# Hypersonic-cpu/DSP-AudioRecLabs

Hardware: AMD Instinct MI355X
Metric: frames/sec (framing+window+E/M/ZCR) on 1 s 44.1 kHz clips; 1/2/4/8 GPU (higher is better)
Workload: dtype fp32

## Files before the change

dsp-audioreclabs_amd/csrc/extract.hip:

```cpp
#include <hip/hip_runtime.h>
#include <stdint.h>

#include <algorithm>

#include "dsp_audiorec.h"
#include "extract_layout.h"
#include "dsp_device.h"

#ifndef DSP_ABL
#define DSP_ABL 0
#endif

namespace dsp {

static constexpr int NT = EXTRACT_THREADS;
static constexpr int NWAVE = NT / 64;
static constexpr int RREG = EXTRACT_RREG;
static constexpr int NRV = 4 * RREG;

#ifdef DSP_STAMPS
#define STAMP(clip, k)                                                                           \
    do {                                                                                         \
        if (threadIdx.x == 0 && p.stamps) p.stamps[(size_t)(clip) * 32 + (k)] = __builtin_amdgcn_s_memtime(); \
    } while (0)
// ... 26 lines not shown
#define MARK(name) \
    do {           \
    } while (0)
#endif

struct ExtractParams {
    const int16_t *pcm;
    const int64_t *offsets;
    int B, ncap, L, S;
    const double *window;
    int do_vad;
    double hi, lo, zr;
    float *feat;
    int32_t *start_end, *n_frames, *status;
    int ostride;
    double *vad_energy;
    int32_t *vad_zcr;
    int ld_vad;
    float *seq;
    int ld_seq;
    unsigned long long *stamps;
    unsigned *queue;
    int qchunk;
    ExtractCarve cv;
};

static_assert(__is_standard_layout(ExtractParams) && __is_trivially_copyable(ExtractParams),
              "ExtractParams is a plain kernel argument block");
static_assert(sizeof(ExtractParams) <= 1024, "kernel argument block");

struct ClipStatsRaw {
    double mq, Mp, invM2;
    float invMf;
    int tpos, t0, nv, kneg;
};
struct Shared {
    long long red_k[NWAVE];
    int red_a[NWAVE], red_b[NWAVE];
    double pa, pb;
    ClipStatsRaw cs;
    double noise_e, noise_z;
    double oslo[3], oshi[3];
    int n3, n1, n6, exact, j0, j1, next;
    int qnext, qend, qcursor, qrange;
    int cdir, cy;
    unsigned smask;
    int schunk;
    int sclear;
    long long noff[2];
    int noff_for;
};
static_assert(sizeof(Shared) <= EXTRACT_SHARED_BYTES, "grow EXTRACT_SHARED_BYTES");
static_assert((EXTRACT_OSTAGE & (EXTRACT_OSTAGE - 1)) == 0 && EXTRACT_OSTAGE <= 32, "chunk of 2^k <= 32 clips");

struct ClipRef {
    int64_t base;
    int lead, n, nvec, nword;
    bool ok;
};

__device__ __forceinline__ ClipRef clip_ref_at(const ExtractParams &p, int64_t o0, int64_t o1)
{
    ClipRef c;
    const int64_t nn = o1 - o0;
    c.ok = nn > 0 && nn <= p.ncap;
    c.n = c.ok ? (int)nn : 0;
    c.base = o0 & ~(int64_t)7;
    c.lead = (int)(o0 - c.base);
    c.nvec = c.ok ? (c.lead + c.n + 7) >> 3 : 0;
    c.nword = (c.lead + c.n + 31) >> 5;
    return c;
}
__device__ __forceinline__ ClipRef clip_ref(const ExtractParams &p, int i)
{
    return clip_ref_at(p, p.offsets[i], p.offsets[i + 1]);
}
__device__ __forceinline__ ClipRef clip_none()
{
    ClipRef c;
    c.base = 0;
    c.lead = c.n = c.nvec = c.nword = 0;
    c.ok = false;
    return c;
}

struct Ctx {
    Shared *sh;
    const float *wtab;
    uint32_t *posw;
    unsigned long long *wS2;
    int *wS1;
    double *vE;
    int32_t *vZ;
    float *fE, *fM;
    int32_t *fZ;
    uint16_t *zw;
    int *ztot;
    int *rank;
    int *pS1;
    unsigned long long *pS2;
    int32_t *orow;
    int64_t total;
    int stamp_clip;
};

__device__ __forceinline__ __amdgpu_buffer_rsrc_t clip_rsrc(const ExtractParams &p, const ClipRef &c)
{
    return __builtin_amdgcn_make_buffer_rsrc(const_cast<int16_t *>(p.pcm + c.base), 0, c.nvec * 16, 0x00020000);
}
__device__ __forceinline__ short8 load_vec(const ExtractParams &p, const ClipRef &c, int v)
{
    return __builtin_bit_cast(short8, __builtin_amdgcn_raw_buffer_load_b128(clip_rsrc(p, c), 16 * v, 0, 0));
}
__device__ __forceinline__ short8 load_cvec(const ExtractParams &p, const ClipRef &c, int v)
{
    return __builtin_bit_cast(short8, __builtin_amdgcn_raw_buffer_load_b128(clip_rsrc(p, c), 2 * c.lead + 16 * v, 0, 0));
}
__device__ __forceinline__ void issue_clip(short8 (&regs)[NRV], const ExtractParams &p, const ClipRef &c,
                                           int tid = (int)threadIdx.x, int r0 = 0, int r1 = RREG)
{
    const __amdgpu_buffer_rsrc_t rs = clip_rsrc(p, c);
    const int voff = 64 * tid;
#pragma unroll
    for (int r = r0; r < r1; r++)
#pragma unroll
        for (int k = 0; k < 4; k++)
            regs[4 * r + k] = __builtin_bit_cast(
                short8, __builtin_amdgcn_raw_buffer_load_b128(rs, voff + 16 * k, 64 * NT * r, 0));
}
__device__ __forceinline__ int opaque_tid()
{
    int t = (int)threadIdx.x;
    asm volatile("" : "+v"(t));
    return t;
}

__device__ __forceinline__ void vad_noise(const Ctx &c, int nv, int lane)
{
    const double *vE = c.vE;
    const int32_t *vZ = c.vZ;
    const int nfr = min(5, nv / 10);
    double noise_e, noise_z;
    if (nfr > 0) {
        long long zs = 0;
        for (int q = 0; q < nfr; q++) zs += vZ[q] + vZ[nv - nfr + q];
        auto cat = [&](int q) { return q < nfr ? vE[q] : vE[nv - 2 * nfr + q]; };
        noise_e = np_small_sum(cat, 2 * nfr) / (double)(2 * nfr);
        noise_z = (double)zs / (double)(2 * nfr);
    } else {
        double me = INFINITY;
        int mz = 0x7fffffff;
        for (int q = lane; q < nv; q += 64) {
            me = fmin(me, vE[q]);
            mz = min(mz, vZ[q]);
        }
        noise_e = wave_mind(me);
        noise_z = (double)wave_min(mz);
    }
    if (lane == 0) {
        c.sh->noise_e = noise_e;
        c.sh->noise_z = noise_z;
    }
}

template <bool CERTIFY, bool FAST>
__device__ __forceinline__ int vad_scan(const ExtractParams &p, const Ctx &c, int nv, int lane)
{
    const double *vE = c.vE;
    const int32_t *vZ = c.vZ;
    Shared *sh = c.sh;
    const double noise_e = sh->noise_e, noise_z = sh->noise_z;
    const double g = p90_weight(nv);
    const double p90 = np_lerp(sh->pa, sh->pb, g);
    const ExtractParams &q = p;
    const VadThresholds th = vad_thresholds(p90, noise_e, noise_z, q);
    const double t1 = th.t1, t2 = th.t2, tz = th.tz;
    STAMP(c.stamp_clip, 10);
    int flag = 0, n3 = -1, n1 = 0, n6 = nv - 1;
    auto short_scan = [&](auto kc_t) {
        constexpr int KC = decltype(kc_t)::value;
        BitsK<KC> hiE, loE, loZ, nr1, nr2;
#pragma unroll
        for (int k = 0; k < KC; k++) {
            const int q = 64 * k + lane;
            const bool in = q < nv;
            const double e = in ? vE[q] : 0.0;
            const int z = in ? vZ[q] : 0;
            hiE.w[k] = __ballot(in && e > t1);
            loE.w[k] = __ballot(in && e <= t2);
            loZ.w[k] = __ballot(in && (double)z <= tz);
            nr1.w[k] = CERTIFY ? __ballot(in && near_tie(e, t1)) : 0ull;
            nr2.w[k] = CERTIFY ? __ballot(in && near_tie(e, t2)) : 0ull;
        }
        n3 = bits_first_ge(hiE, 0);
        const int n4 = bits_last_lt(hiE, nv);
        if (CERTIFY) {
            if (n3 < 0) flag |= bits_any_in(nr1, 0, nv);
            else flag |= bits_any_in(nr1, 0, n3 + 1) || bits_any_in(nr1, n4, nv);
        }
        if (n3 >= 0) {
            const int b2 = bits_last_lt(loE, n3);
            const int n2 = b2 >= 0 ? b2 + 1 : 0;
            const int b5 = bits_first_ge(loE, n4 + 1);
            const int n5 = b5 >= 0 ? b5 - 1 : nv - 1;
            if (CERTIFY)
                flag |= bits_any_in(nr2, max(n2 - 1, 0), n3) || bits_any_in(nr2, n4 + 1, min(n5 + 2, nv));
            const int b1 = bits_last_lt(loZ, n2);
            n1 = b1 >= 0 ? b1 + 1 : 0;
            const int b6 = bits_first_ge(loZ, n5 + 1);
            n6 = b6 >= 0 ? b6 - 1 : nv - 1;
        }
    };
    if (FAST || nv <= 128) {
        short_scan(IntT<2>());
    } else if (nv <= 256) {
        short_scan(IntT<4>());
    } else {
        int n4 = -1;
        for (int q0 = 0; q0 < nv; q0 += 64) {
            const int f = q0 + lane;
            const unsigned long long m = __ballot(f < nv && vE[f] > t1);
            if (m) {
                if (n3 < 0) n3 = q0 + __ffsll((long long)m) - 1;
                n4 = q0 + 63 - __clzll((long long)m);
            }
        }
        if (CERTIFY)
            for (int q0 = 0; q0 < nv; q0 += 64) {
                const int f = q0 + lane;
                const bool chk = f < nv && (n3 < 0 || f <= n3 || f >= n4);
                if (__ballot(chk && near_tie(vE[f], t1))) flag = 1;
            }
        if (n3 >= 0) {
            int n2 = 0, n5 = nv - 1;
            for (int q0 = ((n3 - 1) >> 6) << 6; q0 >= 0 && n3 > 0; q0 -= 64) {
                const int q = q0 + lane;
                const unsigned long long m = __ballot(q < n3 && vE[q] <= t2);
                if (m) {
                    n2 = q0 + 63 - __clzll((long long)m) + 1;
                    break;
                }
            }
            for (int q0 = ((n4 + 1) >> 6) << 6; q0 < nv; q0 += 64) {
                const int q = q0 + lane;
                const unsigned long long m = __ballot(q > n4 && q < nv && vE[q] <= t2);
                if (m) {
                    n5 = q0 + __ffsll((long long)m) - 2;
                    break;
                }
            }
            if (CERTIFY)
                for (int q0 = 0; q0 < nv; q0 += 64) {
                    const int q = q0 + lane;
                    const bool chk = q < nv && ((q >= n2 - 1 && q < n3) || (q > n4 && q <= n5 + 1));
                    if (__ballot(chk && near_tie(vE[q], t2))) flag = 1;
                }
            for (int q0 = ((n2 - 1) >> 6) << 6; q0 >= 0 && n2 > 0; q0 -= 64) {
                const int q = q0 + lane;
                const unsigned long long m = __ballot(q < n2 && (double)vZ[q] <= tz);
                if (m) {
                    n1 = q0 + 63 - __clzll((long long)m) + 1;
                    break;
                }
            }
            for (int q0 = ((n5 + 1) >> 6) << 6; q0 < nv; q0 += 64) {
                const int q = q0 + lane;
                const unsigned long long m = __ballot(q > n5 && q < nv && (double)vZ[q] <= tz);
                if (m) {
                    n6 = q0 + __ffsll((long long)m) - 2;
                    break;
                }
            }
        }
    }
    if (lane == 0) {
        sh->n3 = n3;
        sh->n1 = n1;
        sh->n6 = n6;
    }
    STAMP(c.stamp_clip, 11);
    return flag;
}

__device__ __forceinline__ int vad_partial_word(const ClipRef &cur, int L, int S, int nv, int t, int &e0, int &e1)
{
    e0 = e1 = 0;
    if (t >= 2 * nv) return -1;
    const int f = t >> 1;
    const bool end = t & 1;
    const int u0 = cur.lead + f * S, u1 = u0 + L;
    const int wa = u0 >> 5, wb = (u1 - 1) >> 5;
    if (!end && (u0 & 31)) {
        e0 = u0 & 31;
        e1 = min(32, u1 - 32 * wa);
        return wa;
    }
    if (end && (u1 & 31) && (wb != wa || !(u0 & 31))) {
        e0 = max(0, u0 - 32 * wb);
        e1 = u1 & 31;
        return wb;
    }
    return -1;
}
__device__ __forceinline__ void partial_moments_fast(const short8 (&q)[4], int e0, int e1, bool kneg, int &t1,
                                                     unsigned long long &t2)
{
    const uint32_t hi = e1 >= 32 ? ~0u : (1u << e1) - 1u;
    const uint32_t M = hi & ~((1u << e0) - 1u);
    const short2v ones = {1, 1};
    int s1 = 0;
    unsigned long long s2 = 0;
#pragma unroll
    for (int k = 0; k < 4; k++) {
        const uint32_t Mk = M >> (8 * k);
        short2v dm[4];
#pragma unroll
        for (int h = 0; h < 4; h++) {
            const uint32_t b0 = (uint32_t)__builtin_amdgcn_sbfe((int)Mk, 2 * h, 1);
            const uint32_t b1 = (uint32_t)__builtin_amdgcn_sbfe((int)Mk, 2 * h + 1, 1);
            const uint32_t m = (b0 & 0x0000FFFFu) | (b1 & 0xFFFF0000u);
            dm[h] = __builtin_bit_cast(short2v, __builtin_bit_cast(uint32_t, half_pair(q[k], h)) & m);
            s1 = __builtin_amdgcn_sdot2(dm[h], ones, s1, false);
        }
        if (kneg) {
#pragma unroll
            for (int h = 0; h < 4; h++) s2 += (unsigned)sq2(dm[h]);
        } else {
            s2 += (unsigned)sq2acc(dm[1], sq2(dm[0]));
            s2 += (unsigned)sq2acc(dm[3], sq2(dm[2]));
        }
    }
    t1 += s1;
    t2 += s2;
}

__device__ __forceinline__ int uni(int v) { return __builtin_amdgcn_readfirstlane(v); }
__device__ __forceinline__ float uni(float v)
{
    return __builtin_bit_cast(float, __builtin_amdgcn_readfirstlane(__builtin_bit_cast(int, v)));
}
__device__ __forceinline__ double uni(double v)
{
    const long long b = __builtin_bit_cast(long long, v);
    const unsigned lo = __builtin_amdgcn_readfirstlane((int)b), hi = __builtin_amdgcn_readfirstlane((int)(b >> 32));
    return __builtin_bit_cast(double, (long long)(((unsigned long long)hi << 32) | lo));
}

__device__ __forceinline__ uint64_t uni_u64(uint64_t v)
{
    const unsigned lo = __builtin_amdgcn_readfirstlane((int)v), hi = __builtin_amdgcn_readfirstlane((int)(v >> 32));
    return ((uint64_t)hi << 32) | lo;
}

struct R1Acc {
    int K, kmin, kmax;
    short2v pmin, pmax;
};
__device__ __forceinline__ R1Acc r1_acc_init()
{
    R1Acc a;
    a.K = 0;
    a.kmin = 0x7fffffff;
    a.kmax = -0x7fffffff - 1;
    a.pmin = (short2v){32767, 32767};
    a.pmax = (short2v){-32768, -32768};
    return a;
}
__device__ __forceinline__ void r1_interior(const short8 *q, int w, R1Acc &a, int *wS1, unsigned long long *wS2)
{
    int s1 = 0;
    unsigned long long s2 = 0;
    const short2v ones = {1, 1};
#pragma unroll
    for (int k = 0; k < 4; k++)
#pragma unroll
        for (int h = 0; h < 4; h += 2) {
            const short2v d0 = half_pair(q[k], h), d1 = half_pair(q[k], h + 1);
            a.pmin = __builtin_elementwise_min(a.pmin, d0);
            a.pmax = __builtin_elementwise_max(a.pmax, d0);
            a.pmin = __builtin_elementwise_min(a.pmin, d1);
            a.pmax = __builtin_elementwise_max(a.pmax, d1);
            s1 = __builtin_amdgcn_sdot2(d0, ones, s1, false);
            s1 = __builtin_amdgcn_sdot2(d1, ones, s1, false);
            s2 += (unsigned)sq2acc(d1, sq2(d0));
        }
    wS1[w] = s1;
    wS2[w] = s2;
    a.K += s1;
}
__device__ __forceinline__ void r1_redo_s2(const short8 *q, int w, unsigned long long *wS2)
{
    unsigned long long s2 = 0;
#pragma unroll
    for (int k = 0; k < 4; k++)
#pragma unroll
        for (int h = 0; h < 4; h++) s2 += (unsigned)sq2(half_pair(q[k], h));
    wS2[w] = s2;
}
__device__ __forceinline__ int r1_edge_issue(const ExtractParams &p, const ClipRef &cur, int lane)
{
    const int w = lane < 32 ? 0 : cur.nword - 1, u = 32 * w + (lane & 31);
    const bool valid = (lane < 32 || cur.nword > 1) && u >= cur.lead && u < cur.lead + cur.n;
    const int x = (short)__builtin_amdgcn_raw_buffer_load_b16(clip_rsrc(p, cur), valid ? 2 * u : 0x40000000, 0, 0);
    return valid ? x : 0x7fffffff;
}
__device__ __forceinline__ void r1_edges(int xv, int nword, int lane, R1Acc &a, int *wS1, unsigned long long *wS2)
{
    const bool valid = xv != 0x7fffffff;
    const int x = valid ? xv : 0;
    if (valid) {
        a.kmin = min(a.kmin, x);
        a.kmax = max(a.kmax, x);
    }
    a.K += x;
    const int w = lane < 32 ? 0 : nword - 1;
    if ((lane & 31) == 0 && (lane == 0 || nword > 1)) {
        int z1 = 0;
        unsigned long long z2 = 0;
        asm volatile("" : "+v"(z1), "+v"(z2));
        wS1[w] = z1;
        wS2[w] = z2;
    }
    if (valid) {
        __hip_atomic_fetch_add(wS1 + w, x, __ATOMIC_RELAXED, __HIP_MEMORY_SCOPE_WORKGROUP);
        __hip_atomic_fetch_add(wS2 + w, (unsigned long long)(unsigned)(x * x), __ATOMIC_RELAXED,
                               __HIP_MEMORY_SCOPE_WORKGROUP);
    }
}
__device__ __forceinline__ void r1_reduce_rows(const R1Acc &a, const Ctx &c, int wid, int lane)
{
    const int kmn = min(a.kmin, min((int)a.pmin.x, (int)a.pmin.y));
    const int kmx = max(a.kmax, max((int)a.pmax.x, (int)a.pmax.y));
    const int ks = dpp_row_reduce(a.K, OpAdd()), rmn = dpp_row_reduce(kmn, OpMin()), rmx = dpp_row_reduce(kmx, OpMax());
    if ((lane & 15) == 0) {
        int *rk = reinterpret_cast<int *>(c.vE);
        const int slot = 4 * wid + (lane >> 4);
        rk[slot] = ks;
        rk[32 + slot] = rmn;
        rk[64 + slot] = rmx;
    }
}
__device__ __forceinline__ uint32_t neg_byte255(const short8 &val, short2v tt, uint32_t acc)
{
    unsigned a[4];
#pragma unroll
    for (int h = 0; h < 4; h++) a[h] = __builtin_bit_cast(unsigned, __builtin_elementwise_sub_sat(half_pair(val, h), tt));
    const unsigned s03 = __builtin_amdgcn_perm(a[1], a[0], 0x0B0A0908u);
    const unsigned s47 = __builtin_amdgcn_perm(a[3], a[2], 0x0B0A0908u);
    return __builtin_amdgcn_udot4(s47, 0x80402010u, __builtin_amdgcn_udot4(s03, 0x08040201u, acc, false), false);
}
__device__ __forceinline__ uint32_t pos_word(const short8 *q, int w, int nword, int lead, int n, int tpos)
{
    const bool tbig = tpos > 32767;
    const short2v tt = {(short)(tbig ? 32767 : tpos), (short)(tbig ? 32767 : tpos)};
    const uint32_t x0 = neg_byte255(q[0], tt, 255u), x1 = neg_byte255(q[1], tt, 0u), x2 = neg_byte255(q[2], tt, 0u),
                   x3 = neg_byte255(q[3], tt, 0u);
    uint32_t P = tbig ? 0u : ((((x3 << 8) + x2) << 8) + x1 << 8) + x0;
    P = tbig ? 0u : P * 0x01010101u;
    if (w == 0 || w == nword - 1) {
        const int lo_ = min(max(lead - 32 * w, 0), 32), hi_ = min(max(lead + n - 32 * w, 0), 32);
        const uint32_t mhi = hi_ >= 32 ? ~0u : ((1u << hi_) - 1u);
        const uint32_t mlo = lo_ >= 32 ? 0u : ~((1u << lo_) - 1u);
        P &= mhi & mlo;
    }
    return P;
}

__device__ __forceinline__ int wave_incl_scan(int v)
{
    v += __builtin_amdgcn_update_dpp(0, v, 0x111, 0xF, 0xF, true);
    v += __builtin_amdgcn_update_dpp(0, v, 0x112, 0xF, 0xF, true);
    v += __builtin_amdgcn_update_dpp(0, v, 0x114, 0xF, 0xF, true);
    v += __builtin_amdgcn_update_dpp(0, v, 0x118, 0xF, 0xF, true);
    v += __builtin_amdgcn_update_dpp(0, v, 0x142, 0xA, 0xF, false);
    v += __builtin_amdgcn_update_dpp(0, v, 0x143, 0xC, 0xF, false);
    return v;
}
__device__ __forceinline__ void zseg_word(const uint16_t *zw_, const int *zt_, uint32_t P, int w, int lane, int seg)
{
    uint16_t *zw = const_cast<uint16_t *>(zw_);
    int *ztot = const_cast<int *>(zt_);
    const uint32_t nb = (uint32_t)__builtin_amdgcn_update_dpp(0, (int)P, 0x130, 0xF, 0xF, true);
    uint32_t ch = P ^ ((P >> 1) | (nb << 31));
    if (lane == 63) ch &= 0x7fffffffu;
    const int cz = __popc(ch), inc = wave_incl_scan(cz);
    zw[w] = (uint16_t)(inc - cz);
    if (lane == 63) ztot[seg] = inc;
}
__device__ __forceinline__ int zseg_count(const uint32_t *posw, const uint16_t *zw, const int *ztot, int x0, int x1)
{
    if (x1 <= x0) return 0;
    const int w0 = x0 >> 5, w1 = x1 >> 5, s0 = w0 >> 6;
    int cnt = (int)zw[w1] - (int)zw[w0] - __popc(chg_word(posw, w0) & ((1u << (x0 & 31)) - 1u));
    if (x1 & 31) cnt += __popc(chg_word(posw, w1) & ((1u << (x1 & 31)) - 1u));
    if ((w1 >> 6) != s0) cnt += ztot[s0] + (int)(chg_word(posw, 64 * s0 + 63) >> 31);
    return cnt;
}

struct ClipStats {
    double mq, Mp, invM2;
    float invMf;
    int tpos, t0, nv;
    int kneg;
};
__device__ __forceinline__ ClipStats clip_stats_rows(const Ctx &c, int lane, int n, int L, int S, int do_vad)
{
    const int *rk = reinterpret_cast<const int *>(c.vE);
    const int K = wave_sum(lane < 32 ? rk[lane] : 0);
    const int kmin = wave_min(lane < 32 ? rk[32 + lane] : 0x7fffffff);
    const int kmax = wave_max(lane < 32 ? rk[64 + lane] : -0x7fffffff - 1);
    ClipStats s;
    s.mq = uni((double)K / (double)n);
    s.Mp = uni(fmax((double)kmax - s.mq, s.mq - (double)kmin));
    s.tpos = uni((int)floor(s.mq) + 1);
    s.t0 = uni((int)floor(s.mq + 0.5));
    s.invMf = uni(s.Mp > 0.0 ? (float)(1.0 / s.Mp) : 0.0f);
    s.invM2 = uni(s.Mp > 0.0 ? 1.0 / (s.Mp * s.Mp) : 0.0);
    s.nv = (do_vad && n >= L) ? (n - L) / S + 1 : 0;
    s.kneg = kmin == -32768;
    return s;
}

__device__ __forceinline__ void p90_select_wave(const Ctx &c, int nv, int lane)
{
    const P90Rank<int> pr = p90_rank(nv);
    const int r0 = pr.r0, r1 = pr.r1;
    const bool in0 = lane < nv, in1 = lane + 64 < nv;
    const unsigned long long f0 = in0 ? dkey(c.vE[lane]) : 0ull;
    const unsigned long long f1 = in1 ? dkey(c.vE[lane + 64]) : 0ull;
    const unsigned o0 = (unsigned)(f0 >> 32), o1 = (unsigned)(f1 >> 32);
    const int d1 = nv - 1 - r1, d0 = nv - 1 - r0;
    unsigned h0 = o0, h1 = o1, ka = 0, kb = 0;
    for (int t = 0;; t++) {
        const unsigned m = wave_reduce(h0 > h1 ? h0 : h1, OpMax());
        if (t == d1) kb = m;
        if (t == d0) {
            ka = m;
            break;
        }
        const unsigned long long b0 = __ballot(h0 == m);
        if (b0) {
            if (lane == __ffsll((long long)b0) - 1) h0 = 0u;
        } else {
            if (lane == __ffsll((long long)__ballot(h1 == m)) - 1) h1 = 0u;
        }
    }
    auto full_at = [&](int r) -> double {
        const unsigned kh = r == r0 ? ka : kb;
        const unsigned long long c0 = __ballot(in0 && o0 == kh), c1 = __ballot(in1 && o1 == kh);
        if (__popcll(c0) + __popcll(c1) == 1)
            return dkey_value(c0 ? lane_read(f0, __ffsll((long long)c0) - 1)
                                 : lane_read(f1, __ffsll((long long)c1) - 1));
        const int rr = r - (__popcll(__ballot(in0 && o0 < kh)) + __popcll(__ballot(in1 && o1 < kh)));
        unsigned long long res = 0;
        for (int hh = 0; hh < 2; hh++) {
            unsigned long long cm = hh ? c1 : c0;
            while (cm) {
                const int l = __ffsll((long long)cm) - 1;
                cm &= cm - 1;
                const unsigned long long e = lane_read(hh ? f1 : f0, l);
                const int lt = __popcll(__ballot(in0 && o0 == kh && f0 < e)) + __popcll(__ballot(in1 && o1 == kh && f1 < e));
                const int eq = __popcll(__ballot(in0 && f0 == e)) + __popcll(__ballot(in1 && f1 == e));
                if (rr >= lt && rr < lt + eq) res = e;
            }
        }
        return dkey_value(res);
    };
    const double pa = full_at(r0), pb = full_at(r1);
    if (lane == 0) {
        c.sh->pa = pa;
        c.sh->pb = pb;
    }
}

__device__ __forceinline__ int vad_partial_issue(const ExtractParams &p, const ClipRef &cur, int L, int S, int nv,
                                                 int t, short8 (&qa)[4], int &e0, int &e1)
{
    const int pw = vad_partial_word(cur, L, S, nv, t, e0, e1);
    const __amdgpu_buffer_rsrc_t rs = clip_rsrc(p, cur);
    const int off = pw >= 0 ? 64 * pw : 0x40000000;
#pragma unroll
    for (int k = 0; k < 4; k++)
        qa[k] = __builtin_bit_cast(short8, __builtin_amdgcn_raw_buffer_load_b128(rs, off + 16 * k, 0, 0));
    return pw;
}

__device__ __forceinline__ void vad_frames_fast(const Ctx &c, const ClipRef &cur, int L, int S, const ClipStats &cs,
                                                const short8 (&qa)[4], int pa_w, int pa_e0, int pa_e1, int tid)
{
    const int nv = cs.nv, lead = cur.lead;
    const int f = tid >> 1, lh = tid & 1;
    const bool act = f < nv;
    int s1 = 0;
    unsigned long long s2 = 0;
    int zc = 0;
    if (act) {
        const int u0 = lead + f * S, u1 = u0 + L;
        const int wa = u0 >> 5, wb = (u1 - 1) >> 5;
        const int wi0 = (u0 & 31) ? wa + 1 : wa, wi1 = (u1 & 31) ? wb - 1 : wb;
        const int per = (wi1 - wi0 + 2) >> 1;
        const int ws = wi0 + lh * per, we = min(ws + per - 1, wi1);
#pragma unroll 4
        for (int w = ws; w <= we && !(DSP_ABL & 32); w++) {
            s1 += c.wS1[w];
            s2 += c.wS2[w];
        }
        zc = (lh || (DSP_ABL & 32)) ? 0 : zseg_count(c.posw, c.zw, c.ztot, u0, u1 - 1);
        if (pa_w >= 0 && !(DSP_ABL & 8)) partial_moments_fast(qa, pa_e0, pa_e1, cs.kneg, s1, s2);
    }
    s1 += dpp_i(s1, DPP_QXOR1);
    {
        const unsigned lo = dpp_i((int)(unsigned)s2, DPP_QXOR1), hi = dpp_i((int)(unsigned)(s2 >> 32), DPP_QXOR1);
        s2 += ((unsigned long long)hi << 32) | lo;
    }
    zc += dpp_i(zc, DPP_QXOR1);
    if (act && lh == 0) {
        c.vE[f] = energy_from_moments(s2, s1, L, cs.t0, cs.mq - (double)cs.t0, cs.invM2);
        c.vZ[f] = zc;
    }
}

static constexpr int R4_KV = 7;
__device__ __forceinline__ int crop_frame_count(int m, int L, int S) { return (m <= L) ? 1 : (m - L + S - 1) / S + 1; }
template <bool ZSEG>
__device__ __forceinline__ int r4_frames(const ExtractParams &p, const Ctx &c, const ClipRef &cur, int L, int S,
                                         int st, int en, const ClipStats &cs, int j0, int j1, int wrank, int lane)
{
    const int n = cur.n, lead = cur.lead;
    const int m = en - st;
    const int F = crop_frame_count(m, L, S);
    const float sE = cs.invMf * cs.invMf, sM = cs.invMf;
    const int wrow = EXTRACT_WROW(L);
    const CanonX cx = canon_x(cs.mq, cs.t0);
    const int vfix = ((lead & 1) && ((lead + n) & 7) == 0) ? (n - 1) >> 3 : -1;
    const short klast = vfix >= 0 ? load_vec(p, cur, cur.nvec - 1)[7] : (short)0;
    auto frame_vec = [&](auto padded_t, auto near_t, const short8 &x8, const float *wr, int jb, int lim,
                         float2v &ea, float &m0, float &m1) {
        constexpr bool PADDED = decltype(padded_t)::value, NEAR0 = decltype(near_t)::value;
        const float4 wa = *reinterpret_cast<const float4 *>(wr + jb);
        const float4 wb = *reinterpret_cast<const float4 *>(wr + jb + 4);
        const float wv[8] = {wa.x, wa.y, wa.z, wa.w, wb.x, wb.y, wb.z, wb.w};
#pragma unroll
        for (int h = 0; h < 4; h++) {
            float2v w = {wv[2 * h], wv[2 * h + 1]};
            if (PADDED) {
                const int j = jb + 2 * h;
                w.x = j < lim ? w.x : 0.f;
                w.y = j + 1 < lim ? w.y : 0.f;
            }
            canon_pair(w, canon_x2<NEAR0>(x8[2 * h], x8[2 * h + 1], cx), ea, m0, m1);
        }
    };
    constexpr int KV = R4_KV;
    const int rl = lane & 15, row = lane >> 4;
    for (int gi = wrank; !(DSP_ABL & 1) && 4 * gi < F; gi += NWAVE) {
        const int g = 4 * gi + row;
        const bool act = g < F;
        const int gc = act ? g : F - 1;
        const int fs = st + gc * S;
        const int lim = min(L, en - fs);
        const bool padded = lim < L;
        const int va = fs >> 3, vb = (fs + lim - 1) >> 3;
        const int r = fs & 3;
        const float *wr = c.wtab + r * wrow + EXTRACT_WPAD + r;
        float2v ea = {0.f, 0.f};
        float m0 = 0.f, m1 = 0.f;
        for (int v0 = va; v0 <= vb; v0 += 16 * KV) {
            const int vl = v0 + rl, vlim = vb - vl;
            short8 xv[KV];
#pragma unroll
            for (int k = 0; k < KV; k++) xv[k] = load_cvec(p, cur, vl + 16 * k);
            if (vfix >= 0)
#pragma unroll
                for (int k = 0; k < KV; k++)
                    if (vl + 16 * k == vfix) xv[k][(n - 1) & 7] = klast;
            const int jl = 8 * vl - fs;
            auto run = [&](auto pt, auto nt, auto ft) {
#pragma unroll
                for (int k = 0; k < KV; k++)
                    if (decltype(ft)::value || 16 * k <= vlim) frame_vec(pt, nt, xv[k], wr, jl + 128 * k, lim, ea, m0, m1);
            };
            const bool full = !padded && __all(vlim >= 16 * (KV - 1));
            if (padded)
                cx.near0 ? run(BoolT<true>(), BoolT<true>(), BoolT<false>()) : run(BoolT<true>(), BoolT<false>(), BoolT<false>());
            else if (cx.near0)
                full ? run(BoolT<false>(), BoolT<true>(), BoolT<true>()) : run(BoolT<false>(), BoolT<true>(), BoolT<false>());
            else
                full ? run(BoolT<false>(), BoolT<false>(), BoolT<true>()) : run(BoolT<false>(), BoolT<false>(), BoolT<false>());
        }
        const float E1 = dpp_row_reduce(ea.x + ea.y, OpAdd()) * sE;
        const float M1 = dpp_row_reduce(m0 + m1, OpAdd()) * sM;
        const int ia = fs + j0, ib = min(fs + j1, en - 1);
        int z = 0;
        if constexpr (!ZSEG) {
            z = dpp_row_reduce(ia < ib ? chg_count(c.posw, ia + lead, ib + lead, rl, 16) : 0, OpAdd());
            if (ia <= ib) {
                if (j0 > 0) z += pos_bit(c.posw, ia + lead);
                if (ib < fs + L - 1) z += pos_bit(c.posw, ib + lead);
            }
        }
        if (act && rl == 0) {
            c.fE[g] = E1;
            c.fM[g] = M1;
            if constexpr (!ZSEG) c.fZ[g] = z;
        }
    }
    return F;
}
__device__ __forceinline__ void crop_zcr(const Ctx &c, int lead, int L, int S, int st, int en, int F, int j0, int j1,
                                         int lane)
{
    for (int g = lane; !(DSP_ABL & 1) && g < F; g += 64) {
        const int fs = st + g * S;
        const int ia = fs + j0, ib = min(fs + j1, en - 1);
        int z = 0;
        if (ia <= ib) {
            z = zseg_count(c.posw, c.zw, c.ztot, ia + lead, ib + lead);
            if (j0 > 0) z += pos_bit(c.posw, ia + lead);
            if (ib < fs + L - 1) z += pos_bit(c.posw, ib + lead);
        }
        c.fZ[g] = z;
    }
}

__device__ __forceinline__ void r5_small(const Ctx &c, int F, float *featb, int wid, int lane)
{
    if (wid >= 4 || (DSP_ABL & 2)) return;
    const int r0 = (F - 1) / 2, r1 = F / 2;
    const int hl = lane & 31;
    const bool up = lane >= 32, zjob = wid & 1;
    const bool in = hl < F && !(zjob && up);
    float x = 0.f;
    if (in) x = zjob ? (float)c.fZ[hl] : up ? c.fM[hl] : c.fE[hl];
    const int q = zjob ? 2 : (up ? 1 : 0);
    if (wid < 2) {
        if (DSP_ABL & 256) return;
        unsigned b[1] = {in ? fkey(x) : ~0u};
        wave_bitonic<1, unsigned, 32>(b, lane);
        const float a0 = fkey_value(lane_read(b[0], r0)), a1 = fkey_value(lane_read(b[0], r1));
        const float u0 = fkey_value(lane_read(b[0], 63 - r0)), u1 = fkey_value(lane_read(b[0], 63 - r1));
        const float v0 = up ? u0 : a0, v1 = up ? u1 : a1;
        double med;
        {
#pragma clang fp contract(off)
            med = (F & 1) ? (double)v1 : ((double)v0 + (double)v1) / 2.0;
        }
        if (hl == 0 && !(zjob && up)) featb[5 * q + 4] = (float)med;
    } else {
        if (DSP_ABL & 512) return;
        const double Fd = (double)F;
        const double rs = dpp_row_reduce(in ? (double)x : 0.0, OpAdd());
        const float rmx = dpp_row_reduce(in ? x : -INFINITY, OpMax()), rmn = dpp_row_reduce(in ? x : INFINITY, OpMin());
        const double mean_lo = (lane_read(rs, 0) + lane_read(rs, 16)) / Fd, mean_hi = (lane_read(rs, 32) + lane_read(rs, 48)) / Fd;
        const double d = in ? (double)x - (up ? mean_hi : mean_lo) : 0.0;
        const double rq = dpp_row_reduce(__builtin_fma(d, d, 0.0), OpAdd());
        const double qq_lo = lane_read(rq, 0) + lane_read(rq, 16), qq_hi = lane_read(rq, 32) + lane_read(rq, 48);
        const float mx_lo = OpMax()(lane_read(rmx, 0), lane_read(rmx, 16)), mx_hi = OpMax()(lane_read(rmx, 32), lane_read(rmx, 48));
        const float mn_lo = OpMin()(lane_read(rmn, 0), lane_read(rmn, 16)), mn_hi = OpMin()(lane_read(rmn, 32), lane_read(rmn, 48));
        if (lane < (zjob ? 4 : 8)) {
            const bool h = lane >= 4;
            const int k = lane & 3;
            const double o = k == 0 ? (h ? mean_hi : mean_lo) : k == 1 ? sqrt((h ? qq_hi : qq_lo) / Fd)
                             : k == 2 ? (double)(h ? mx_hi : mx_lo) : (double)(h ? mn_hi : mn_lo);
            featb[5 * (zjob ? 2 : (int)h) + k] = (float)o;
        }
    }
}
__device__ __forceinline__ void r5_fast(const Ctx &c, int F, float *featb, int wid, int lane)
{
    const int r0 = (F - 1) / 2, r1 = F / 2;
    for (int job = wid; !(DSP_ABL & 2) && job < 6; job += NWAVE) {
        if ((DSP_ABL & 256) && job < 3) continue;
        if ((DSP_ABL & 512) && job >= 3) continue;
        const int q = job % 3;
        auto get = [&](int j) -> float { return q == 0 ? c.fE[j] : q == 1 ? c.fM[j] : (float)c.fZ[j]; };
        const bool in0 = lane < F, in1 = lane + 64 < F;
        const float x0 = in0 ? get(lane) : 0.f, x1 = in1 ? get(lane + 64) : 0.f;
        if (job < 3) {
            unsigned a[2] = {in0 ? fkey(x0) : ~0u, in1 ? fkey(x1) : ~0u};
            float v0, v1;
            if (F <= 32) {
                unsigned b[1] = {a[0]};
                wave_bitonic<1, unsigned, 32>(b, lane);
                v0 = fkey_value(sorted_at<1>(b, r0));
                v1 = fkey_value(sorted_at<1>(b, r1));
            } else if (F <= 64) {
                unsigned b[1] = {a[0]};
                wave_bitonic<1>(b, lane);
                v0 = fkey_value(sorted_at<1>(b, r0));
                v1 = fkey_value(sorted_at<1>(b, r1));
            } else {
                wave_bitonic<2>(a, lane);
                v0 = fkey_value(sorted_at<2>(a, r0));
                v1 = fkey_value(sorted_at<2>(a, r1));
            }
            double med;
            {
#pragma clang fp contract(off)
                med = (F & 1) ? (double)v1 : ((double)v0 + (double)v1) / 2.0;
            }
            if (lane == 0) featb[5 * q + 4] = (float)med;
        }
        if (job >= 3) {
            const double s = wave_sum((in0 ? (double)x0 : 0.0) + (in1 ? (double)x1 : 0.0));
            const float mx = wave_reduce(fmaxf(in0 ? x0 : -INFINITY, in1 ? x1 : -INFINITY), OpMax());
            const float mn = wave_reduce(fminf(in0 ? x0 : INFINITY, in1 ? x1 : INFINITY), OpMin());
            const double mean = s / (double)F;
            const double d0 = in0 ? (double)x0 - mean : 0.0, d1 = in1 ? (double)x1 - mean : 0.0;
            const double qq = wave_sum(fma(d0, d0, d1 * d1));
            if (lane < 4) {
                const double o = lane == 0 ? mean : lane == 1 ? sqrt(qq / (double)F) : lane == 2 ? (double)mx
                                 : (double)mn;
                featb[5 * q + lane] = (float)o;
            }
        }
    }
}
static constexpr int XCD_RANGES = 8;
static constexpr int QSTRIDE = 64;
static_assert(11 * QSTRIDE * 4 <= DSP_QUEUE_WS_BYTES, "queue_ws too small for the counter layout");
__device__ __forceinline__ unsigned *qword(unsigned *q, int w) { return q + w * QSTRIDE; }
struct ClipQueue {
    unsigned *q;
    int B, nch, xcd, ch;
    int s0;
};
__device__ __forceinline__ ClipQueue queue_open(const ExtractParams &p, Shared *sh)
{
    ClipQueue Q;
    Q.q = p.qchunk > 0 ? p.queue : nullptr;
    Q.B = p.B;
    Q.ch = max(p.qchunk, 1);
    Q.nch = (p.B + Q.ch - 1) / Q.ch;
    Q.s0 = min(Q.nch, (int)gridDim.x);
    Q.xcd = __builtin_amdgcn_s_getreg((3 << 11) | 20) & 7;
    if (threadIdx.x == 0) {
        const int b = (int)blockIdx.x;
        sh->qnext = b < Q.nch ? b * Q.ch : 0;
        sh->qend = b < Q.nch ? min(Q.B, b * Q.ch + Q.ch) : 0;
        sh->qrange = 0;
        sh->qcursor = (int)blockIdx.x - (int)gridDim.x;
    }
    return Q;
}
__device__ __forceinline__ unsigned queue_begin(const ClipQueue &Q, Shared *sh)
{
    if (!Q.q) {
        const int t = sh->qcursor + (int)gridDim.x;
        sh->qcursor = t;
        sh->cdir = t < Q.B ? t : -1;
        return 0;
    }
    const int nx = sh->qnext;
    if (nx < sh->qend) {
        sh->qnext = nx + 1;
        sh->cdir = nx;
        return 0;
    }
    if (sh->qrange >= XCD_RANGES || Q.s0 == Q.nch) {
        sh->cdir = -1;
        return 0;
    }
    const int y = (Q.xcd + sh->qrange) % XCD_RANGES;
    sh->cy = y;
    sh->cdir = -2;
    return __hip_atomic_fetch_add(qword(Q.q, y), 1u, __ATOMIC_RELAXED, __HIP_MEMORY_SCOPE_AGENT);
}
__device__ __forceinline__ int queue_end(const ClipQueue &Q, Shared *sh, unsigned ret)
{
    constexpr int NR = XCD_RANGES;
    if (sh->cdir != -2) return sh->cdir;
    int y = sh->cy;
    for (;;) {
        const int D = Q.nch - Q.s0;
        const int c0 = Q.s0 + y * D / NR, c1 = Q.s0 + (y + 1) * D / NR;
        const int r0 = c0 * Q.ch, r1 = min(Q.B, c1 * Q.ch);
        const int nbig = max(0, r1 - r0 - 2 * ((int)gridDim.x / NR)) / Q.ch;
        const int first = (int)ret < nbig ? r0 + (int)ret * Q.ch : r0 + nbig * Q.ch + ((int)ret - nbig);
        if ((int)ret < nbig || first < r1) {
            sh->qnext = first + 1;
            sh->qend = (int)ret < nbig ? first + Q.ch : first + 1;
            return first;
        }
        int r = ++sh->qrange;
        if (r >= NR) return -1;
        y = (Q.xcd + r) % NR;
        ret = __hip_atomic_fetch_add(qword(Q.q, y), 1u, __ATOMIC_RELAXED, __HIP_MEMORY_SCOPE_AGENT);
    }
}
__device__ __forceinline__ int queue_next(const ClipQueue &Q, Shared *sh) { return queue_end(Q, sh, queue_begin(Q, sh)); }
__device__ __forceinline__ void queue_done(const ExtractParams &p)
{
    if (!p.queue) return;
    const unsigned d = __hip_atomic_fetch_add(qword(p.queue, 8), 1u, __ATOMIC_ACQ_REL, __HIP_MEMORY_SCOPE_AGENT);
    if (d == gridDim.x - 1) {
#pragma unroll
        for (int y = 0; y < 8; y++) __hip_atomic_store(qword(p.queue, y), 0u, __ATOMIC_RELAXED, __HIP_MEMORY_SCOPE_AGENT);
        __hip_atomic_store(qword(p.queue, 8), 0u, __ATOMIC_RELEASE, __HIP_MEMORY_SCOPE_AGENT);
    }
}

__device__ __forceinline__ void stamp_loads_landed(const ExtractParams &p, int i, int wid, int lane)
{
#ifdef DSP_STAMPS
    if (p.stamps) {
        asm volatile("s_waitcnt vmcnt(0)" ::: "memory");
        STAMP(i, 13);
        if (lane == 0) p.stamps[(size_t)i * 32 + 24 + wid] = __builtin_amdgcn_s_memtime();
    }
#endif
}
__device__ __forceinline__ void reset_staged(Shared *sh, int tid)
{
    if (tid == 0 && sh->sclear) {
        sh->smask = 0;
        sh->schunk = -1;
        sh->sclear = 0;
    }
}
__device__ __forceinline__ void share_clip_stats(Shared *sh, const ClipStats &c0, int lane)
{
    if (lane == 0) sh->cs = {c0.mq, c0.Mp, c0.invM2, c0.invMf, c0.tpos, c0.t0, c0.nv, c0.kneg};
}
__device__ __forceinline__ ClipStats shared_clip_stats(const Shared *sh)
{
    ClipStats cs;
    cs.mq = uni(sh->cs.mq);
    cs.Mp = uni(sh->cs.Mp);
    cs.invM2 = uni(sh->cs.invM2);
    cs.invMf = uni(sh->cs.invMf);
    cs.tpos = uni(sh->cs.tpos);
    cs.t0 = uni(sh->cs.t0);
    cs.nv = uni(sh->cs.nv);
    cs.kneg = uni(sh->cs.kneg);
    return cs;
}
__device__ __forceinline__ void crop_from_scan(const Shared *sh, int L, int S, int n, int &st, int &en)
{
    if (sh->n3 >= 0) {
        st = sh->n1 * S;
        en = min(sh->n6 * S + L, n);
    }
}
__device__ __forceinline__ void dump_vad(const ExtractParams &p, const Ctx &c, int i, int nv)
{
    if (p.vad_energy)
        for (int f = opaque_tid(); f < nv && f < p.ld_vad; f += NT) {
            p.vad_energy[(size_t)i * p.ld_vad + f] = c.vE[f];
            p.vad_zcr[(size_t)i * p.ld_vad + f] = c.vZ[f];
        }
}
__device__ __forceinline__ void stage_outputs(const Ctx &c, int i, int st, int en, int F)
{
    Shared *sh = c.sh;
    const int oslot = i & (EXTRACT_OSTAGE - 1);
    int32_t *orow = c.orow + DSP_OUT_ROW_WORDS * oslot;
    orow[15] = st;
    orow[16] = en;
    orow[17] = F;
    orow[18] = DSP_CLIP_OK;
    const int ch = i / EXTRACT_OSTAGE;
    const unsigned m0 = sh->schunk == ch ? sh->smask : 0u;
    sh->schunk = ch;
    sh->smask = m0 | (1u << oslot);
}


template <typename Resolve>
__device__ __forceinline__ bool clip_fast(const ExtractParams &p, const Ctx &c, int i, const ClipRef &cur,
                                          short8 (&regs)[NRV], Resolve resolve)
{
    Shared *sh = c.sh;
    const int tid = opaque_tid(), lane = tid & 63, wid = __builtin_amdgcn_readfirstlane(tid >> 6);
    int L = p.L, S = p.S;
    asm volatile("" : "+s"(L), "+s"(S));
    const int n = cur.n, lead = cur.lead, nword = cur.nword;
    const int oslot = i & (EXTRACT_OSTAGE - 1);
    float *featb = reinterpret_cast<float *>(c.orow + DSP_OUT_ROW_WORDS * oslot);
    STAMP(i, 0);
    stamp_loads_landed(p, i, wid, lane);

    MARK(R1);
    R1Acc acc = r1_acc_init();
#pragma unroll
    for (int r = 0; r < RREG; r++) {
        const int w = r * NT + tid;
        if (w < nword && w > 0 && w < nword - 1) r1_interior(&regs[4 * r], w, acc, c.wS1, c.wS2);
    }
    if (wid == NWAVE - 1) r1_edges(r1_edge_issue(p, cur, lane), nword, lane, acc, c.wS1, c.wS2);
    MARK(R1red);
    r1_reduce_rows(acc, c, wid, lane);
    __syncthreads();
    reset_staged(sh, tid);
    MARK(stats);
    if (wid == 0) share_clip_stats(sh, clip_stats_rows(c, lane, n, L, S, p.do_vad), lane);
    __syncthreads();
    const ClipStats cs = shared_clip_stats(sh);
    const int nv = cs.nv;
    STAMP(i, 1);

    MARK(R2);
    if (cs.kneg) {
#pragma unroll
        for (int r = 0; r < RREG; r++) {
            const int w = r * NT + tid;
            if (w < nword && w > 0 && w < nword - 1) r1_redo_s2(&regs[4 * r], w, c.wS2);
        }
    }
    uint32_t P[RREG];
#pragma unroll
    for (int r = 0; r < RREG; r++) {
        const int w = r * NT + tid;
        P[r] = (w < nword && !(DSP_ABL & 4)) ? pos_word(&regs[4 * r], w, nword, lead, n, cs.tpos) : 0u;
        if (w < nword) c.posw[w] = P[r];
    }
#pragma unroll
    for (int r = 0; r < RREG && !(DSP_ABL & 16); r++) zseg_word(c.zw, c.ztot, P[r], r * NT + tid, lane, r * NWAVE + wid);
    if (tid < 2) c.posw[nword + tid] = 0;
    if (tid == 0) c.zw[RREG * NT] = 0;
    MARK(paissue);
    short8 qa[4];
    int pa_e0 = 0, pa_e1 = 0, pa_w = -1;
    if (64 * wid < 2 * nv)
        pa_w = vad_partial_issue(p, cur, L, S, nv, tid, qa, pa_e0, pa_e1);
    __syncthreads();
    STAMP(i, 2);

    MARK(passAB);
    if (nv > 0) {
        vad_frames_fast(c, cur, L, S, cs, qa, pa_w, pa_e0, pa_e1, tid);
        STAMP(i, 7);
        __syncthreads();
        STAMP(i, 8);
        MARK(p90);
        if (wid == 0) {
            __builtin_amdgcn_s_setprio(2);
            if (DSP_ABL & 64) {
                const double mx = wave_maxd(fmax(lane < nv ? c.vE[lane] : 0.0, lane + 64 < nv ? c.vE[lane + 64] : 0.0));
                if (lane == 0) sh->pa = sh->pb = 0.8 * mx;
            } else {
                p90_select_wave(c, nv, lane);
            }
        }
        if (wid == 1) vad_noise(c, nv, lane);
        __syncthreads();
        STAMP(i, 3);
        MARK(scan);
        if (wid == 0) {
            int flag = 0;
            if (DSP_ABL & 128) {
                if (lane == 0) {
                    sh->n3 = 0;
                    sh->n1 = nv / 3;
                    sh->n6 = min(nv / 3 + 25, nv - 1);
                }
            } else {
                flag = vad_scan<true, true>(p, c, nv, lane);
            }
            if (lane == 0) sh->exact = cs.Mp > 0.0 ? flag : 0;
        }
    }
    MARK(resolve);
    if (tid == 0) sh->next = resolve();
    if (wid == 0) __builtin_amdgcn_s_setprio(0);
    __syncthreads();
    int st = 0, en = n;
    if (nv > 0) {
        if (sh->exact) return false;
        crop_from_scan(sh, L, S, n, st, en);
        dump_vad(p, c, i, nv);
    }
    STAMP(i, 4);

    MARK(R4);
    if (wid == NWAVE - 1) crop_zcr(c, lead, L, S, st, en, crop_frame_count(en - st, L, S), sh->j0, sh->j1, lane);
    const int F = r4_frames<true>(p, c, cur, L, S, st, en, cs, sh->j0, sh->j1, wid, lane);
    STAMP(i, 12);
    __syncthreads();
    STAMP(i, 5);

    MARK(R5);
    if (const int Fu = uni(F); Fu <= 32) r5_small(c, Fu, featb, wid, lane);
    else r5_fast(c, Fu, featb, wid, lane);
    if (wid == NWAVE - 1) {
        const int nx = sh->next;
        if (nx >= 0 && lane < 2) sh->noff[lane] = p.offsets[nx + lane];
        if (lane == 0) sh->noff_for = nx;
    }
    STAMP(i, 9);
    MARK(tail);
    const ExtractParams &qs = p;
    if (qs.seq)
        for (int g = tid; g < F && g < qs.ld_seq; g += NT) {
            float *o = qs.seq + ((size_t)i * qs.ld_seq + g) * 3;
            o[0] = c.fE[g];
            o[1] = c.fM[g];
            o[2] = (float)c.fZ[g];
        }
    if (tid == 0) stage_outputs(c, i, st, en, F);
    STAMP(i, 6);
    return true;
}

__device__ __forceinline__ void write_bad_clip(const ExtractParams &p, int i, int tid)
{
    if (tid < 15) out_feat(p, i)[tid] = __builtin_nanf("");
    if (tid == 0) {
        const int64_t nn = p.offsets[i + 1] - p.offsets[i];
        *out_st(p, i) = nn <= 0 ? DSP_CLIP_EMPTY : DSP_CLIP_TOO_LONG;
        int z = 0;
        asm volatile("" : "+v"(z));
        out_se(p, i)[0] = z;
        out_se(p, i)[1] = z;
        *out_nf(p, i) = 0;
    }
}


__device__ __forceinline__ Ctx ctx_from(const ExtractCarve &cv, unsigned char *lds)
{
    Ctx c;
    c.sh = reinterpret_cast<Shared *>(lds + cv.sh);
    c.wtab = reinterpret_cast<const float *>(lds + cv.wtab);
    c.posw = reinterpret_cast<uint32_t *>(lds + cv.posw);
    c.wS2 = reinterpret_cast<unsigned long long *>(lds + cv.wS2);
    c.wS1 = reinterpret_cast<int *>(lds + cv.wS1);
    c.vE = reinterpret_cast<double *>(lds + cv.vE);
    c.vZ = reinterpret_cast<int32_t *>(lds + cv.vZ);
    c.fE = reinterpret_cast<float *>(lds + cv.fE);
    c.fM = reinterpret_cast<float *>(lds + cv.fM);
    c.fZ = reinterpret_cast<int32_t *>(lds + cv.fZ);
    c.rank = reinterpret_cast<int *>(lds + cv.rank);
    c.zw = reinterpret_cast<uint16_t *>(lds + cv.zw);
    c.ztot = reinterpret_cast<int *>(lds + cv.ztot);
    c.pS1 = reinterpret_cast<int *>(lds + cv.pS1);
    c.pS2 = reinterpret_cast<unsigned long long *>(lds + cv.pS2);
    c.orow = reinterpret_cast<int32_t *>(lds + cv.ost);
    c.total = 0;
    c.stamp_clip = 0;
    return c;
}
template <bool FAST>
__device__ __forceinline__ Ctx make_ctx(const ExtractParams &p, unsigned char *lds)
{
    if constexpr (FAST) {
        constexpr ExtractCarve cv = extract_carve_fast();
        return ctx_from(cv, lds);
    } else {
        return ctx_from(p.cv, lds);
    }
}

__device__ __forceinline__ void build_window(const ExtractParams &p, const Ctx &c, int tid, int lane, int wid)
{
    float *wt = const_cast<float *>(c.wtab);
    Shared *sh = c.sh;
    const int L = p.L;
    constexpr int WPRE = 3;
    double wv[WPRE];
#pragma unroll
    for (int k = 0; k < WPRE; k++) {
        const int j = tid + NT * k;
        wv[k] = j < L ? p.window[j] : 0.0;
    }
    if (tid == 0) {
        sh->j0 = L;
        sh->j1 = -1;
    }
    const int wrow = EXTRACT_WROW(L);
    for (int t = tid; t < 4 * (wrow - L); t += NT) {
        const int r = t / (wrow - L), q = t - r * (wrow - L);
        wt[r * wrow + (q < EXTRACT_WPAD + r ? q : q + L)] = 0.f;
    }
    __syncthreads();
    auto put_weight = [&](int q0, double w) {
        const int j = q0 + lane;
        const bool in = j < L;
        if (in) {
#pragma unroll
            for (int r = 0; r < 4; r++) wt[r * wrow + j + EXTRACT_WPAD + r] = (float)w;
        }
        const unsigned long long m = __ballot(in && w > 0.0);
        if (lane == 0 && m) {
            atomicMin(&sh->j0, q0 + __ffsll((long long)m) - 1);
            atomicMax(&sh->j1, q0 + 63 - __clzll((long long)m));
        }
    };
#pragma unroll
    for (int k = 0; k < WPRE; k++) put_weight(NT * k + wid * 64, wv[k]);
    for (int q0 = NT * WPRE + wid * 64; q0 < L; q0 += NT) put_weight(q0, q0 + lane < L ? p.window[q0 + lane] : 0.0);
    __syncthreads();
}


__device__ __forceinline__ void flush_outputs(const ExtractParams &p, const Ctx &c, int done, int tid)
{
    constexpr int CH = EXTRACT_OSTAGE, RW = DSP_OUT_ROW_WORDS;
    const int cb = done & ~(CH - 1);
    const unsigned m = c.sh->schunk == cb / CH ? c.sh->smask : 0u;
    if (tid < RW * CH) {
        const int j = tid / RW, col = tid - RW * j;
        if ((m >> j) & 1) {
            const int32_t v = c.orow[tid];
            int32_t *dst = col < 15   ? (int32_t *)out_feat(p, cb + j) + col
                           : col < 17 ? out_se(p, cb + j) + (col - 15)
                           : col == 17 ? out_nf(p, cb + j)
                                       : out_st(p, cb + j);
            *dst = v;
        }
    }
}



}

#include "extract_generic.h"

namespace dsp {

template <bool FAST>
__global__ __launch_bounds__(NT) __attribute__((amdgpu_waves_per_eu(2 * (FAST ? EXTRACT_WG_PER_CU : EXTRACT_WG_PER_CU_GENERIC))))
void extract_kernel(ExtractParams p)
{
    extern __shared__ __attribute__((aligned(16))) unsigned char lds[];
    Ctx c = make_ctx<FAST>(p, lds);
    Shared *sh = c.sh;
    const int tid = threadIdx.x, lane = tid & 63, wid = __builtin_amdgcn_readfirstlane(tid >> 6);
    WG_STAMP(16);
    short8 regs[NRV];
    if constexpr (FAST) {
        const int b = (int)blockIdx.x, ch = max(p.qchunk, 1);
        const int first = (p.qchunk > 0 && p.queue) ? (b < (p.B + ch - 1) / ch ? b * ch : -1) : (b < p.B ? b : -1);
        const ClipRef c0 = first >= 0 ? clip_ref(p, first) : clip_none();
        issue_clip(regs, p, c0.ok ? c0 : clip_none(), opaque_tid());
    }
    build_window(p, c, tid, lane, wid);
    WG_CK(18);
    const ClipQueue Q = queue_open(p, sh);
    if (tid == 0) {
        sh->next = queue_next(Q, sh);
        sh->smask = 0;
        sh->schunk = -1;
        sh->sclear = 0;
        sh->noff_for = -1;
    }
    __syncthreads();
    WG_CK(19);
    bool inflight = false;
    for (int i = sh->next; i >= 0;) {
        STAMP(i, 20);
#ifdef DSP_STAMPS
        if (threadIdx.x == 0 && p.stamps) p.stamps[(size_t)i * 32 + 21] = blockIdx.x;
#endif
        MARK(looptop);
        const ClipRef cur = (FAST && sh->noff_for == i) ? clip_ref_at(p, sh->noff[0], sh->noff[1]) : clip_ref(p, i);
        if (!cur.ok) {
            __syncthreads();
            if (tid == 0) sh->next = queue_next(Q, sh);
            write_bad_clip(p, i, opaque_tid());
            inflight = false;
        } else {
            if (!FAST && !inflight) issue_clip(regs, p, cur, opaque_tid());
            unsigned cl = 0;
            if (tid == 0) cl = queue_begin(Q, sh);
            c.stamp_clip = i;
            bool done;
            if constexpr (FAST) {
                done = clip_fast(p, c, i, cur, regs, [&]() { return queue_end(Q, sh, cl); });
            } else {
                done = clip_body<false>(p, c, i, cur, regs, [&]() { return queue_end(Q, sh, cl); });
                if (!done && tid == 0) sh->next = queue_end(Q, sh, cl);
            }
            if (!done && tid == 0) {
                *out_st(p, i) = DSP_CLIP_UNCERTIFIED;
                if (p.queue) __hip_atomic_fetch_add(qword(p.queue, 9), 1u, __ATOMIC_RELAXED, __HIP_MEMORY_SCOPE_AGENT);
            }
            inflight = !FAST && done;
        }
        MARK(loopbot);
        __syncthreads();
        STAMP(i, 14);
        const int prev = i;
        i = sh->next;
        if (i < 0 || (i ^ prev) >= EXTRACT_OSTAGE) {
            flush_outputs(p, c, prev, opaque_tid());
            if (tid == 0) sh->sclear = 1;
        }
        if constexpr (FAST) {
            ClipRef nx = i < 0 ? clip_none() : sh->noff_for == i ? clip_ref_at(p, sh->noff[0], sh->noff[1]) : clip_ref(p, i);
            if (!nx.ok) nx = clip_none();
            nx.base = (int64_t)uni_u64((uint64_t)nx.base);
            nx.nvec = uni(nx.nvec);
            issue_clip(regs, p, nx, opaque_tid());
        }
        STAMP(prev, 15);
    }
    if (tid == 0) queue_done(p);
    WG_STAMP(22);
}

__global__ __launch_bounds__(NT) void extract_exact_kernel(ExtractParams p)
{
    if (p.queue && __hip_atomic_load(qword(p.queue, 9), __ATOMIC_RELAXED, __HIP_MEMORY_SCOPE_AGENT) == 0u) return;
    extern __shared__ __attribute__((aligned(16))) unsigned char lds[];
    Ctx c = make_ctx<false>(p, lds);
    Shared *sh = c.sh;
    const int tid = threadIdx.x, lane = tid & 63, wid = __builtin_amdgcn_readfirstlane(tid >> 6);
    int *list = reinterpret_cast<int *>(lds + p.cv.total);
    bool built = false;
    for (int64_t b0 = 0; b0 < p.B; b0 += (int64_t)gridDim.x * NT) {
        const int64_t i = b0 + blockIdx.x + (int64_t)gridDim.x * tid;
        const bool tie = i < p.B && *out_st(p, (int)i) == DSP_CLIP_UNCERTIFIED;
        if (tid == 0) sh->next = 0;
        __syncthreads();
        if (tie) list[atomicAdd(&sh->next, 1)] = (int)i;
        __syncthreads();
        const int nt = sh->next;
        for (int t = 0; t < nt; t++) {
            const int ci = list[t];
            if (!built) {
                build_window(p, c, tid, lane, wid);
                built = true;
            }
            c.stamp_clip = ci;
            const ClipRef cr = clip_ref(p, ci);
            short8 regs[NRV];
            issue_clip(regs, p, cr);
            clip_body<true>(p, c, ci, cr, regs);
            __syncthreads();
        }
    }
    if (p.queue && tid == 0) {
// ... 110 lines not shown
```

Before: 5.532 billion.

## Halve VAD partial-word loads and compute boundary moments by subtraction

Frame boundary partial moments now come from a 32-byte half-word load instead of a full 64-byte word. The code sums whole words including the boundary words, then subtracts the excluded part, using the complement from the per-word totals when the loaded half is the wrong one. Mask construction swaps sbfe sequences for a shifted-bitmask multiply and dot. The load issue is also hoisted above the pos/zseg word computation so its latency overlaps that work. This lowers global load bytes and VGPR pressure, at the cost of extra shared-memory reads and more complex edge-case logic.

```diff
diff --git a/dsp-audioreclabs_amd/csrc/extract.hip b/dsp-audioreclabs_amd/csrc/extract.hip
--- a/dsp-audioreclabs_amd/csrc/extract.hip
+++ b/dsp-audioreclabs_amd/csrc/extract.hip
@@ -352,25 +352,30 @@
     }
     return -1;
 }
-__device__ __forceinline__ void partial_moments_fast(const short8 (&q)[4], int e0, int e1, bool kneg, int &t1,
-                                                     unsigned long long &t2)
-{
-    const uint32_t hi = e1 >= 32 ? ~0u : (1u << e1) - 1u;
-    const uint32_t M = hi & ~((1u << e0) - 1u);
-    const short2v ones = {1, 1};
+__device__ __forceinline__ int frame_end_pos(int lead, int L, int S, int t)
+{
+    return lead + (int)__umul24((unsigned)(t >> 1), (unsigned)S) + ((t & 1) ? L - 1 : 0);
+}
+typedef unsigned short ushort2v __attribute__((ext_vector_type(2)));
+__device__ __forceinline__ void partial_moments_half(const short8 (&q)[2], int w, int e, int lead, int n, bool kneg,
+                                                     int &p1, unsigned long long &p2)
+{
+    const bool hi = e > 16;
+    const int r0 = w == 0 ? lead : 0, r1 = min(lead + n - 32 * w, 32);
+    const int a = hi ? e - 16 : r0, b = hi ? min(max(r1 - 16, 0), 16) : min(e, r1);
+    const uint32_t M = ((1u << b) - 1u) & ~((1u << a) - 1u);
+    const uint32_t X = M | (M << 15);
     int s1 = 0;
     unsigned long long s2 = 0;
 #pragma unroll
-    for (int k = 0; k < 4; k++) {
-        const uint32_t Mk = M >> (8 * k);
+    for (int k = 0; k < 2; k++) {
         short2v dm[4];
 #pragma unroll
         for (int h = 0; h < 4; h++) {
-            const uint32_t b0 = (uint32_t)__builtin_amdgcn_sbfe((int)Mk, 2 * h, 1);
-            const uint32_t b1 = (uint32_t)__builtin_amdgcn_sbfe((int)Mk, 2 * h + 1, 1);
-            const uint32_t m = (b0 & 0x0000FFFFu) | (b1 & 0xFFFF0000u);
-            dm[h] = __builtin_bit_cast(short2v, __builtin_bit_cast(uint32_t, half_pair(q[k], h)) & m);
-            s1 = __builtin_amdgcn_sdot2(dm[h], ones, s1, false);
+            const uint32_t wt = (X >> (8 * k + 2 * h)) & 0x00010001u;
+            const short2v d = half_pair(q[k], h);
+            s1 = __builtin_amdgcn_sdot2(d, __builtin_bit_cast(short2v, wt), s1, false);
+            dm[h] = __builtin_bit_cast(short2v, __builtin_bit_cast(ushort2v, d) * __builtin_bit_cast(ushort2v, wt));
         }
         if (kneg) {
 #pragma unroll
@@ -380,8 +385,8 @@
             s2 += (unsigned)sq2acc(dm[3], sq2(dm[2]));
         }
     }
-    t1 += s1;
-    t2 += s2;
+    p1 = s1;
+    p2 = s2;
 }
 
 __device__ __forceinline__ int uni(int v) { return __builtin_amdgcn_readfirstlane(v); }
@@ -623,40 +628,51 @@
     }
 }
 
-__device__ __forceinline__ int vad_partial_issue(const ExtractParams &p, const ClipRef &cur, int L, int S, int nv,
-                                                 int t, short8 (&qa)[4], int &e0, int &e1)
-{
-    const int pw = vad_partial_word(cur, L, S, nv, t, e0, e1);
+__device__ __forceinline__ int vad_partial_issue(const ExtractParams &p, const ClipRef &cur, int L, int S, bool live,
+                                                 int t, short8 (&qa)[2])
+{
+    const int x = frame_end_pos(cur.lead, L, S, t);
+    const int h = t & 1, e = (x & 31) + h;
     const __amdgpu_buffer_rsrc_t rs = clip_rsrc(p, cur);
-    const int off = pw >= 0 ? 64 * pw : 0x40000000;
-#pragma unroll
-    for (int k = 0; k < 4; k++)
+    const int off = (!live || e == 32 * h) ? 0x40000000 : 2 * (x & ~31) + (e > 16 ? 32 : 0);
+#pragma unroll
+    for (int k = 0; k < 2; k++)
         qa[k] = __builtin_bit_cast(short8, __builtin_amdgcn_raw_buffer_load_b128(rs, off + 16 * k, 0, 0));
-    return pw;
+    return x;
 }
 
 __device__ __forceinline__ void vad_frames_fast(const Ctx &c, const ClipRef &cur, int L, int S, const ClipStats &cs,
-                                                const short8 (&qa)[4], int pa_w, int pa_e0, int pa_e1, int tid)
-{
-    const int nv = cs.nv, lead = cur.lead;
+                                                const short8 (&qa)[2], int pa_x, int tid)
+{
+    const int nv = cs.nv;
     const int f = tid >> 1, lh = tid & 1;
     const bool act = f < nv;
     int s1 = 0;
     unsigned long long s2 = 0;
     int zc = 0;
     if (act) {
-        const int u0 = lead + f * S, u1 = u0 + L;
+        const int u0 = lh ? pa_x - (L - 1) : pa_x, u1 = u0 + L;
         const int wa = u0 >> 5, wb = (u1 - 1) >> 5;
-        const int wi0 = (u0 & 31) ? wa + 1 : wa, wi1 = (u1 & 31) ? wb - 1 : wb;
-        const int per = (wi1 - wi0 + 2) >> 1;
-        const int ws = wi0 + lh * per, we = min(ws + per - 1, wi1);
+        const int per = (wb - wa + 2) >> 1;
+        const int ws = wa + lh * per, we = min(ws + per - 1, wb);
 #pragma unroll 4
         for (int w = ws; w <= we && !(DSP_ABL & 32); w++) {
             s1 += c.wS1[w];
             s2 += c.wS2[w];
         }
         zc = (lh || (DSP_ABL & 32)) ? 0 : zseg_count(c.posw, c.zw, c.ztot, u0, u1 - 1);
-        if (pa_w >= 0 && !(DSP_ABL & 8)) partial_moments_fast(qa, pa_e0, pa_e1, cs.kneg, s1, s2);
+        if (!(DSP_ABL & 8)) {
+            const int w = lh ? wb : wa, e = (pa_x & 31) + lh;
+            int p1;
+            unsigned long long p2;
+            partial_moments_half(qa, w, e, cur.lead, cur.n, cs.kneg, p1, p2);
+            if ((e > 16) != (bool)lh) {
+                p1 = c.wS1[w] - p1;
+                p2 = c.wS2[w] - p2;
+            }
+            s1 -= p1;
+            s2 -= p2;
+        }
     }
     s1 += dpp_i(s1, DPP_QXOR1);
     {
@@ -1057,6 +1073,12 @@
             if (w < nword && w > 0 && w < nword - 1) r1_redo_s2(&regs[4 * r], w, c.wS2);
         }
     }
+    MARK(paissue);
+    short8 qa[2];
+    int pa_x = 0;
+    if (64 * wid < 2 * nv)
+        pa_x = vad_partial_issue(p, cur, L, S, tid < 2 * nv, tid, qa);
+    MARK(R2bits);
     uint32_t P[RREG];
 #pragma unroll
     for (int r = 0; r < RREG; r++) {
@@ -1068,17 +1090,12 @@
     for (int r = 0; r < RREG && !(DSP_ABL & 16); r++) zseg_word(c.zw, c.ztot, P[r], r * NT + tid, lane, r * NWAVE + wid);
     if (tid < 2) c.posw[nword + tid] = 0;
     if (tid == 0) c.zw[RREG * NT] = 0;
-    MARK(paissue);
-    short8 qa[4];
-    int pa_e0 = 0, pa_e1 = 0, pa_w = -1;
-    if (64 * wid < 2 * nv)
-        pa_w = vad_partial_issue(p, cur, L, S, nv, tid, qa, pa_e0, pa_e1);
     __syncthreads();
     STAMP(i, 2);
 
     MARK(passAB);
     if (nv > 0) {
-        vad_frames_fast(c, cur, L, S, cs, qa, pa_w, pa_e0, pa_e1, tid);
+        vad_frames_fast(c, cur, L, S, cs, qa, pa_x, tid);
         STAMP(i, 7);
         __syncthreads();
         STAMP(i, 8);
```

Measured after the change: 5.627 billion (median of 6 runs). 1.02x the previous value.
